# raulmur/ORB_SLAM2

Measured on NVIDIA H100. Metric: stereo frames/sec (ORB extract L+R + ComputeStereoMatches, KITTI-shaped 1242x375 @2000 kpts), higher is better.
Workload: dtype u8

## Files before the change

### orb_slam2_b200/csrc/borb_host.cu

```cuda
#include <cmath>
#include <cstdarg>
#include <cstdio>
#include <algorithm>
#include <cstdlib>
#include <cstring>

#include "borb_internal.h"

namespace borb {

static thread_local std::string tl_error;
void set_error(const char* fmt, ...) {
    char buf[512];
    va_list ap;
    va_start(ap, fmt);
    vsnprintf(buf, sizeof(buf), fmt, ap);
    va_end(ap);
    tl_error = buf;
}

std::atomic<int> g_poison{-1};

bool allow_max_smem(const void* func) {
    static std::mutex mu;
// ... 150 lines not shown
        v.inv_scale = e->inv_scale[l];
        v.patch_size = (float)(int)(PATCH * e->scale[l]);
        g.blur_base[l] = btile;
        btile += ((v.w + BLUR_TILE_W - 1) / BLUR_TILE_W) * ((v.h + BLUR_TILE_H - 1) / BLUR_TILE_H);
        if (l > 0) {
            const int wpad = (v.w + 8 + 3) & ~3;
            v.xtab_off = (unsigned)(tabs.size() / 4);
            resize_table(g.lv[l - 1].w, v.w, true, wpad - v.w, tabs);
            v.ytab_off = (unsigned)(tabs.size() / 4);
            resize_table(g.lv[l - 1].h, v.h, false, 0, tabs);
            v.xwin_off = (unsigned)(tabs.size() / 4);
            std::vector<int16_t> win;
            v.x_windowed = resize_window_table(tabs, (size_t)v.xtab_off * 4, wpad, win) ? 1 : 0;
            tabs.insert(tabs.end(), win.begin(), win.end());
        }
        if (quadtree_smem_bytes(v.node_cap) > 200 * 1024) {
            set_error("per-level quota %d exceeds the quadtree kernel's shared-memory envelope", v.quota);
            return BORB_ERR_UNSUPPORTED;
        }
    }
    g.blur_base[L] = btile;
    g.blur_tiles = btile;
    g.fast_blocks = blk;
    g.pyr_image_stride = (unsigned)align_up((int)pyr_off, g.lv[0].pitch);
    g.cand_image_stride = cand_off;
    g.sel_image_stride = sel_off;
    if (sel_off >= 65536) { set_error("keypoint capacity %d exceeds 65535", sel_off); return BORB_ERR_UNSUPPORTED; }
    return BORB_OK;
}

void free_workspace(Workspace& ws) {
    cudaFree(ws.pyr); cudaFree(ws.blur); cudaFree(ws.cand); cudaFree(ws.cand_cnt); cudaFree(ws.pnode); cudaFree(ws.sel);
    cudaFree(ws.sel_cnt); cudaFree(ws.kps); cudaFree(ws.desc); cudaFree(ws.nkp); cudaFree(ws.u_right); cudaFree(ws.depth);
    cudaFree(ws.sad); cudaFree(ws.tabs); cudaFree(ws.brief_slots); cudaFree(ws.pair_idx); cudaFree(ws.st_bins); cudaFree(ws.st_recs); cudaFree(ws.stage);
    free(ws.fast_tmaps); cudaFree(ws.fast_tiles);
    ws = Workspace();
}

borb_status ensure(borb_extractor* e, int w, int h, int n_images) {
    if (w < 1 || h < 1 || w > BORB_MAX_DIM || h > BORB_MAX_DIM) { set_error("image size %dx%d outside [1,%d]", w, h, BORB_MAX_DIM); return BORB_ERR_UNSUPPORTED; }
    BORB_CUDA(cudaSetDevice(e->device));
    const bool same_shape = e->have_geom && e->geom.w == w && e->geom.h == h;
    if (same_shape && e->ws.max_images >= n_images) return BORB_OK;
    BORB_CUDA(cudaStreamSynchronize(e->stream));
    std::vector<int16_t> tabs;
    e->have_geom = false;
    e->last_n_images = 0;
    e->last_stereo_pairs = 0;
    borb_status st = build_geometry(e, w, h, tabs);
    if (st != BORB_OK) return st;
    size_t n = (size_t)(n_images > 2 ? n_images : 2);
    if (same_shape && (size_t)e->ws.max_images > n) n = (size_t)e->ws.max_images;
    free_workspace(e->ws);
    if (e->h_counts) { cudaFreeHost(e->h_counts); e->h_counts = nullptr; }
    e->pair_cache.clear();
    const Geometry& g = e->geom;
    Workspace& ws = e->ws;
    BORB_CUDA(cudaMalloc(&ws.pyr, n * g.pyr_image_stride + 256));
    BORB_CUDA(cudaMalloc(&ws.blur, n * g.pyr_image_stride + 256));
    BORB_CUDA(cudaMalloc(&ws.cand, n * g.cand_image_stride * sizeof(uint32_t)));
    BORB_CUDA(cudaMalloc(&ws.pnode, n * g.cand_image_stride * sizeof(int)));
    BORB_CUDA(cudaMalloc(&ws.cand_cnt, n * g.nlevels * sizeof(int)));
    BORB_CUDA(cudaMalloc(&ws.sel, n * g.sel_image_stride * sizeof(uint32_t)));
    BORB_CUDA(cudaMalloc(&ws.sel_cnt, n * g.nlevels * sizeof(int)));
    BORB_CUDA(cudaMalloc(&ws.kps, n * g.sel_image_stride * sizeof(borb_keypoint)));
    BORB_CUDA(cudaMalloc(&ws.desc, n * g.sel_image_stride * 32));
    BORB_CUDA(cudaMalloc(&ws.nkp, n * sizeof(int)));
    BORB_CUDA(cudaMalloc(&ws.u_right, n * g.sel_image_stride * sizeof(float)));
    BORB_CUDA(cudaMalloc(&ws.depth, n * g.sel_image_stride * sizeof(float)));
    BORB_CUDA(cudaMalloc(&ws.sad, n * g.sel_image_stride * sizeof(int)));
    BORB_CUDA(cudaMalloc(&ws.pair_idx, n * 2 * sizeof(int)));
    BORB_CUDA(cudaMalloc(&ws.st_bins, n * stereo_bins_bytes_per_pair()));
    ws.st_recs_bytes = n * (size_t)stereo_rec_stride(g) * stereo_rec_bytes();
    BORB_CUDA(cudaMalloc(&ws.st_recs, ws.st_recs_bytes));
    BORB_CUDA(cudaMalloc(&ws.tabs, (tabs.size() + 4) * sizeof(int16_t)));
    BORB_CUDA(cudaMemcpy(ws.tabs, tabs.data(), tabs.size() * sizeof(int16_t), cudaMemcpyHostToDevice));
    const std::vector<uint32_t>& slots = brief_slot_table();
    BORB_CUDA(cudaMalloc(&ws.brief_slots, slots.size() * sizeof(uint32_t)));
    BORB_CUDA(cudaMemcpy(ws.brief_slots, slots.data(), slots.size() * sizeof(uint32_t), cudaMemcpyHostToDevice));
    BORB_CUDA(cudaMemset(ws.nkp, 0, n * sizeof(int)));
    BORB_CUDA(cudaMallocHost(&e->h_counts, n * 2 * sizeof(int)));
    ws.max_images = (int)n;
    ws.fast_tmaps = malloc(fast_tmaps_bytes());
    if ((st = build_fast_tmaps(g, ws, ws.fast_tmaps)) != BORB_OK) return st;
    if ((st = build_fast_tiles(g, ws)) != BORB_OK) return st;
    e->have_geom = true;
    return BORB_OK;
}

borb_status poison_extract(borb_extractor* e) {
    const int p = poison_byte();
    if (p < 0) return BORB_OK;
    const Geometry& g = e->geom;
    Workspace& ws = e->ws;
    const size_t n = (size_t)ws.max_images;
    cudaStream_t s = e->stream;
    if (ws.stage) BORB_CUDA(cudaMemsetAsync(ws.stage, p, ws.stage_bytes, s));
    BORB_CUDA(cudaMemsetAsync(ws.pyr, p, n * g.pyr_image_stride + 256, s));
    BORB_CUDA(cudaMemsetAsync(ws.blur, p, n * g.pyr_image_stride + 256, s));
    BORB_CUDA(cudaMemsetAsync(ws.cand, p, n * g.cand_image_stride * sizeof(uint32_t), s));
    BORB_CUDA(cudaMemsetAsync(ws.pnode, p, n * g.cand_image_stride * sizeof(int), s));
    BORB_CUDA(cudaMemsetAsync(ws.cand_cnt, p, n * g.nlevels * sizeof(int), s));
    BORB_CUDA(cudaMemsetAsync(ws.sel, p, n * g.sel_image_stride * sizeof(uint32_t), s));
    BORB_CUDA(cudaMemsetAsync(ws.sel_cnt, p, n * g.nlevels * sizeof(int), s));
    BORB_CUDA(cudaMemsetAsync(ws.kps, p, n * g.sel_image_stride * sizeof(borb_keypoint), s));
    BORB_CUDA(cudaMemsetAsync(ws.desc, p, n * g.sel_image_stride * 32, s));
    BORB_CUDA(cudaMemsetAsync(ws.nkp, p, n * sizeof(int), s));
    return BORB_OK;
}

borb_status poison_stereo(borb_extractor* e) {
    const int p = poison_byte();
    if (p < 0) return BORB_OK;
    Workspace& ws = e->ws;
    const size_t n = (size_t)ws.max_images * e->geom.sel_image_stride;
    cudaStream_t s = e->stream;
    BORB_CUDA(cudaMemsetAsync(ws.u_right, p, n * sizeof(float), s));
    BORB_CUDA(cudaMemsetAsync(ws.depth, p, n * sizeof(float), s));
    BORB_CUDA(cudaMemsetAsync(ws.sad, p, n * sizeof(int), s));
    BORB_CUDA(cudaMemsetAsync(ws.st_bins, p, (size_t)ws.max_images * stereo_bins_bytes_per_pair(), s));
    BORB_CUDA(cudaMemsetAsync(ws.st_recs, p, ws.st_recs_bytes, s));
    return BORB_OK;
}

void drain_timing(borb_extractor* e);
void begin_step(borb_extractor* e) {
    if (!e->timing) return;
    if (e->ev.empty()) {
        e->ev.resize((size_t)borb_extractor::EV_RING * 9);
        for (auto& x : e->ev) cudaEventCreate(&x);
    }
    if (e->ev_pending >= borb_extractor::EV_RING) {
        cudaStreamSynchronize(e->stream);
        drain_timing(e);
    }
    e->ev_slot = (e->ev_slot + 1) % borb_extractor::EV_RING;
    e->ev_mask[e->ev_slot] = 0;
    e->ev_pending++;
}
void mark(borb_extractor* e, int i) {
    if (!e->timing || e->ev.empty()) return;
    cudaEventRecord(e->ev[(size_t)e->ev_slot * 9 + i], e->stream);
    e->ev_mask[e->ev_slot] |= 1u << i;
}
void drain_timing(borb_extractor* e) {
    const int R = borb_extractor::EV_RING;
    for (int k = e->ev_pending - 1; k >= 0; k--) {
        const int slot = ((e->ev_slot - k) % R + R) % R;
        const unsigned m = e->ev_mask[slot];
        for (int i = 0; i < 8; i++) {
            float ms = 0.f;
            if (m & (1u << i)) {
                int j = i + 1;
                while (j < 9 && !(m & (1u << j))) j++;
// ... 147 lines not shown
    return BORB_OK;
}

borb_status enqueue_stereo(borb_extractor* eL, borb_extractor* eR, int n_pairs, const int* left_idx, const int* right_idx,
                           float bf, float b) {
    borb_extractor* e = eL;
    const Geometry& g = e->geom;
    std::vector<int> idx(2 * (size_t)n_pairs);
    for (int p = 0; p < n_pairs; p++) {
        idx[2 * p] = left_idx ? left_idx[p] : (eL == eR ? 2 * p : 0);
        idx[2 * p + 1] = right_idx ? right_idx[p] : (eL == eR ? 2 * p + 1 : 0);
        if (idx[2 * p] < 0 || idx[2 * p] >= eL->last_n_images || idx[2 * p + 1] < 0 || idx[2 * p + 1] >= eR->last_n_images) {
            set_error("stereo pair %d refers to an image outside the last batch", p);
            return BORB_ERR_STATE;
        }
    }
    if (n_pairs > e->ws.max_images) { set_error("too many pairs"); return BORB_ERR_INVALID_ARG; }
    if (idx != e->pair_cache) {
        BORB_CUDA(cudaStreamSynchronize(e->stream));
        std::memcpy(e->h_counts, idx.data(), idx.size() * sizeof(int));
        BORB_CUDA(cudaMemcpyAsync(e->ws.pair_idx, e->h_counts, idx.size() * sizeof(int), cudaMemcpyHostToDevice, e->stream));
        e->pair_cache = idx;
    }
    const int rec_stride = stereo_rec_stride(eR->geom);
    const size_t rec_bytes = (size_t)n_pairs * rec_stride * stereo_rec_bytes();
    if (rec_bytes > e->ws.st_recs_bytes) {
        BORB_CUDA(cudaStreamSynchronize(e->stream));
        cudaFree(e->ws.st_recs);
        e->ws.st_recs = nullptr;
        e->ws.st_recs_bytes = 0;
        BORB_CUDA(cudaMalloc(&e->ws.st_recs, rec_bytes));
        e->ws.st_recs_bytes = rec_bytes;
    }
    const borb_status pst = poison_stereo(e);
    if (pst != BORB_OK) return pst;
    StereoView L{eL->ws.pyr, eL->ws.kps, eL->ws.desc, eL->ws.nkp, eL->geom.pyr_image_stride, eL->geom.sel_image_stride};
    StereoView R{eR->ws.pyr, eR->ws.kps, eR->ws.desc, eR->ws.nkp, eR->geom.pyr_image_stride, eR->geom.sel_image_stride};
    mark(e, 6);
    e->launches += launch_stereo(g, L, R, e->ws.pair_idx, n_pairs, bf, b, e->ws.u_right, e->ws.depth, e->ws.sad, g.sel_image_stride,
                                 e->ws.st_bins, e->ws.st_recs, rec_stride, e->stream);
    mark(e, 7);
    BORB_CUDA(cudaGetLastError());
    e->last_stereo_pairs = (eL == eR && !left_idx && !right_idx) ? n_pairs : 0;
    return BORB_OK;
}

borb_status download_stereo(borb_extractor* e, int n_pairs, float* u_right, float* depth, int cap) {
    const Geometry& g = e->geom;
    const int m = cap < g.sel_image_stride ? cap : g.sel_image_stride;
    if (u_right && m > 0)
        BORB_CUDA(cudaMemcpy2DAsync(u_right, (size_t)cap * 4, e->ws.u_right, (size_t)g.sel_image_stride * 4, (size_t)m * 4, n_pairs, cudaMemcpyDeviceToHost, e->stream));
    if (depth && m > 0)
        BORB_CUDA(cudaMemcpy2DAsync(depth, (size_t)cap * 4, e->ws.depth, (size_t)g.sel_image_stride * 4, (size_t)m * 4, n_pairs, cudaMemcpyDeviceToHost, e->stream));
    return BORB_OK;
}

borb_status finish_timing(borb_extractor* e) {
    if (e->timing && e->ev_pending > 0) drain_timing(e);
    return BORB_OK;
}

}

const std::vector<uint32_t>& brief_slot_table() {
    static const std::vector<uint32_t> table = [] {
        std::vector<uint32_t> t((size_t)BRIEF_BINS * 512);
        int row[512], col[512], order[512];
        for (int b = 0; b < BRIEF_BINS; b++) {
            const double th = (b + 0.5) * (2.0 * 3.14159265358979323846 / BRIEF_BINS);
            const double a = std::cos(th), s = std::sin(th);
            for (int p = 0; p < 512; p++) {
                const int x = kPattern[2 * p], y = kPattern[2 * p + 1];
                row[p] = (int)std::lround(x * s + y * a);
// ... 513 lines not shown
```

### orb_slam2_b200/csrc/borb_internal.h

```cpp
#pragma once
#include <cuda_runtime.h>
#include <stdint.h>

#include <atomic>
#include <mutex>
#include <string>
#include <vector>

#include "../../include/borb.h"

namespace borb {

extern std::atomic<int> g_poison;
inline int poison_byte() { return g_poison.load(std::memory_order_relaxed); }

constexpr int EDGE = 19;
constexpr int PATCH = 31;
constexpr int HALF_PATCH = 15;
constexpr int MIN_BORDER = 16;
constexpr int TH_HIGH = 100;
constexpr int TH_LOW = 50;
constexpr int BLUR_TILE_W = 120;
constexpr int BLUR_TILE_H = 64;
constexpr int FAST_TILE_W = 124;
// ... 40 lines not shown
    int ini_th, min_th;
    int fast_mode;
    int fast_blocks;
    unsigned pyr_image_stride;
    unsigned cand_image_stride;
    int sel_image_stride;
    int blur_tiles;
    int blur_base[BORB_MAX_LEVELS + 1];
    int umax[16];
    LevelGeom lv[BORB_MAX_LEVELS];
};

struct Workspace {
    int max_images = 0;
    uint8_t* pyr = nullptr;
    uint8_t* blur = nullptr;
    uint32_t* cand = nullptr;
    int* cand_cnt = nullptr;
    int* pnode = nullptr;
    uint32_t* sel = nullptr;
    int* sel_cnt = nullptr;
    borb_keypoint* kps = nullptr;
    uint8_t* desc = nullptr;
    int* nkp = nullptr;
    float* u_right = nullptr;
    float* depth = nullptr;
    int* sad = nullptr;
    int16_t* tabs = nullptr;
    uint32_t* brief_slots = nullptr;
    int* pair_idx = nullptr;
    int* st_bins = nullptr;
    void* st_recs = nullptr;
    size_t st_recs_bytes = 0;
    uint8_t* stage = nullptr;
    size_t stage_bytes = 0;
    void* fast_tmaps = nullptr;
    void* fast_tiles = nullptr;
    int fast_n_tiles = 0;
};

constexpr int BRIEF_BINS = 32;
const std::vector<uint32_t>& brief_slot_table();

void set_error(const char* fmt, ...);
bool allow_max_smem(const void* func);
#define BORB_CUDA(call)                                                                             \
    do {                                                                                            \
        cudaError_t _e = (call);                                                                    \
        if (_e != cudaSuccess) {                                                                    \
            borb::set_error("%s failed: %s (%s:%d)", #call, cudaGetErrorString(_e), __FILE__, __LINE__); \
            return (_e == cudaErrorNoDevice || _e == cudaErrorInsufficientDriver) ? BORB_ERR_NO_DEVICE : BORB_ERR_CUDA; \
        }                                                                                           \
    } while (0)

int launch_repack_remap(const Geometry& g, const Workspace& ws, const uint8_t* stage, int src_stride, size_t src_image_bytes, int src_w,
                        int src_h, const float* mx0, const float* my0, const float* mx1, const float* my1, int n_images, cudaStream_t s);
int launch_repack_color(const Geometry& g, const Workspace& ws, const uint8_t* stage, int src_stride, size_t src_image_bytes, int channels,
                        int rgb, int n_images, cudaStream_t s);
int launch_repack(const Geometry& g, const Workspace& ws, const uint8_t* stage, int src_stride, size_t src_image_bytes,
                  int n_images, cudaStream_t s);
int launch_pyramid(const Geometry& g, const Workspace& ws, int n_images, cudaStream_t s);
int launch_fast(const Geometry& g, const Workspace& ws, int n_images, cudaStream_t s);
int launch_quadtree(const Geometry& g, const Workspace& ws, int n_images, cudaStream_t s);
int launch_blur(const Geometry& g, const Workspace& ws, int n_images, cudaStream_t s);
int launch_describe(const Geometry& g, const Workspace& ws, int n_images, cudaStream_t s);
int launch_describe_math_probe(int fn, const float* a, const float* b, int n, float* out, cudaStream_t s);
int launch_match_math_probe(int fn, const float* a, const float* b, int n, float log_scale, int n_levels, void* out,
                            cudaStream_t s);

struct StereoView {
    const uint8_t* pyr;
    const borb_keypoint* kps;
    const uint8_t* desc;
    const int* nkp;
    unsigned pyr_image_stride;
    int kp_image_stride;
};
int launch_stereo(const Geometry& g, const StereoView& L, const StereoView& R, const int* d_pair_idx, int n_pairs,
                  float bf, float b, float* d_u_right, float* d_depth, int* d_sad, int out_stride, int* d_bins, void* d_recs,
                  int rec_stride, cudaStream_t s);
int stereo_rec_stride(const Geometry& g);
size_t stereo_bins_bytes_per_pair();
size_t stereo_rec_bytes();
size_t quadtree_smem_bytes(int node_cap);
borb_status build_fast_tmaps(const Geometry& g, const Workspace& ws, void* out_tmaps);
borb_status build_fast_tiles(const Geometry& g, Workspace& ws);
size_t fast_tmaps_bytes();

}

struct borb_extractor {
    borb_extractor_cfg cfg;
    int device = 0;
    cudaStream_t stream = nullptr;
    std::vector<float> scale, inv_scale, sigma2, inv_sigma2;
    std::vector<int> per_level;
    int umax[16];
    bool have_geom = false;
    borb::Geometry geom;
    borb::Workspace ws;
    int last_n_images = 0;
    int last_stereo_pairs = 0;
    int in_channels = 1;
    int in_rgb = 1;
    float* d_map[2][2] = {{nullptr, nullptr}, {nullptr, nullptr}};
    int map_src_w = 0, map_src_h = 0, map_dst_w = 0, map_dst_h = 0;
    int fast_mode = 0;
    uint64_t launches = 0;
    static constexpr int EV_RING = 128;
    bool timing = false;
    std::vector<cudaEvent_t> ev;
    unsigned ev_mask[EV_RING] = {};
    int ev_slot = 0;
    int ev_pending = 0;
    float stage_ms[8] = {};
    double stage_sum_ms[8] = {};
// ... 5 lines not shown
```

### orb_slam2_b200/csrc/k_stereo.cu

```cuda
#include "borb_internal.h"

namespace borb {

namespace {

__device__ __forceinline__ int hamming256(const uint4 a0, const uint4 a1, const uint4* __restrict__ b) {
    const uint4 b0 = b[0], b1 = b[1];
    return __popc(a0.x ^ b0.x) + __popc(a0.y ^ b0.y) + __popc(a0.z ^ b0.z) + __popc(a0.w ^ b0.w) +
           __popc(a1.x ^ b1.x) + __popc(a1.y ^ b1.y) + __popc(a1.z ^ b1.z) + __popc(a1.w ^ b1.w);
}

}

constexpr int SBIN_SHIFT = 3;
constexpr int SBIN_MAX = 512;
struct __align__(16) RightRec { int iR; int band; int octave; float x; };

__global__ void __launch_bounds__(256) stereo_bin_kernel(const __grid_constant__ Geometry g, StereoView Rv,
                                                         const int* __restrict__ pair_idx, int* __restrict__ bin_start,
                                                         RightRec* __restrict__ recs, int rec_stride) {
    __shared__ int cnt[SBIN_MAX + 1];
    __shared__ int wsum[40];
    const int pair = blockIdx.x, tid = threadIdx.x;
    const int imR = pair_idx[2 * pair + 1];
    const int nR = Rv.nkp[imR];
    const int nb = min((g.h >> SBIN_SHIFT) + 1, SBIN_MAX);
    const borb_keypoint* kR = Rv.kps + (size_t)imR * Rv.kp_image_stride;
    for (int i = tid; i <= nb; i += 256) cnt[i] = 0;
    __syncthreads();
    for (int i = tid; i < nR; i += 256) {
        const borb_keypoint kr = kR[i];
        const float r = __fmul_rn(2.0f, g.lv[kr.octave].scale);
        const int maxr = (int)ceilf(__fadd_rn(kr.y, r)), minr = (int)floorf(__fsub_rn(kr.y, r));
        const int b0 = max(minr, 0) >> SBIN_SHIFT, b1 = min(min(maxr, g.h - 1) >> SBIN_SHIFT, nb - 1);
        for (int b = b0; b <= b1; b++) atomicAdd(&cnt[b], 1);
    }
    __syncthreads();
    {
        const int lane = tid & 31, w = tid >> 5;
        const int i0 = 2 * tid, i1 = 2 * tid + 1;
        const int c0 = i0 < nb ? cnt[i0] : 0, c1 = i1 < nb ? cnt[i1] : 0;
        int incl = c0 + c1;
#pragma unroll
        for (int off = 1; off < 32; off <<= 1) {
            const int t = __shfl_up_sync(0xFFFFFFFFu, incl, off);
            if (lane >= off) incl += t;
        }
        if (lane == 31) wsum[w] = incl;
        __syncthreads();
        if (w == 0) {
            int v = lane < 8 ? wsum[lane] : 0, inc2 = v;
#pragma unroll
            for (int off = 1; off < 8; off <<= 1) {
                const int t = __shfl_up_sync(0xFFFFFFFFu, inc2, off);
                if (lane >= off) inc2 += t;
            }
            if (lane < 8) wsum[8 + lane] = inc2 - v;
            if (lane == 7) wsum[16] = inc2;
        }
        __syncthreads();
        const int base = wsum[8 + w] + incl - (c0 + c1);
        if (i0 < nb) cnt[i0] = base;
        if (i1 < nb) cnt[i1] = base + c0;
        if (tid == 0) cnt[nb] = wsum[16];
        __syncthreads();
    }
    int* bs = bin_start + (size_t)pair * (SBIN_MAX + 1);
    for (int i = tid; i <= nb; i += 256) bs[i] = cnt[i];
    __syncthreads();
    RightRec* out = recs + (size_t)pair * rec_stride;
    for (int i = tid; i < nR; i += 256) {
        const borb_keypoint kr = kR[i];
        const float r = __fmul_rn(2.0f, g.lv[kr.octave].scale);
        const int maxr = (int)ceilf(__fadd_rn(kr.y, r)), minr = (int)floorf(__fsub_rn(kr.y, r));
        const int b0 = max(minr, 0) >> SBIN_SHIFT, b1 = min(min(maxr, g.h - 1) >> SBIN_SHIFT, nb - 1);
        RightRec rec;
        rec.iR = i; rec.band = (minr & 0xFFFF) | (maxr << 16); rec.octave = kr.octave; rec.x = kr.x;
        for (int b = b0; b <= b1; b++) {
            const int pos = atomicAdd(&cnt[b], 1);
            if (pos < rec_stride) out[pos] = rec;
        }
    }
}

__global__ void __launch_bounds__(256, 6) stereo_match_kernel(const __grid_constant__ Geometry g, StereoView Lv, StereoView Rv,
                                                           const int* __restrict__ pair_idx, float bf, float b,
                                                           float* __restrict__ u_right, float* __restrict__ depth,
                                                           int* __restrict__ sad, int out_stride,
                                                           const int* __restrict__ bin_start, const RightRec* __restrict__ recs,
                                                           int rec_stride) {
    const int pair = blockIdx.y;
    const int imL = pair_idx[2 * pair], imR = pair_idx[2 * pair + 1];
    const int lane = threadIdx.x & 31;
    const int iL = blockIdx.x * (blockDim.x >> 5) + (threadIdx.x >> 5);
    const int nL = Lv.nkp[imL], nR = Rv.nkp[imR];
    if (iL >= nL) return;
    const size_t o = (size_t)pair * out_stride + iL;
    const borb_keypoint* kL = Lv.kps + (size_t)imL * Lv.kp_image_stride;
    const borb_keypoint* kR = Rv.kps + (size_t)imR * Rv.kp_image_stride;
    const uint8_t* dL = Lv.desc + (size_t)imL * Lv.kp_image_stride * 32;
    const uint8_t* dR = Rv.desc + (size_t)imR * Rv.kp_image_stride * 32;

    float uR_out = -1.0f, depth_out = -1.0f;
    int sad_out = -1;

    const borb_keypoint kp = kL[iL];
    const int levelL = kp.octave;
    const float vL = kp.y, uL = kp.x;
    const float maxD = __fdiv_rn(bf, b);
    const float minU = __fsub_rn(uL, maxD), maxU = uL;
    const int row = (int)vL;
    const uint4 a0 = reinterpret_cast<const uint4*>(dL + (size_t)iL * 32)[0];
    const uint4 a1 = reinterpret_cast<const uint4*>(dL + (size_t)iL * 32)[1];
    unsigned best = ((unsigned)TH_HIGH << 16);
    if (!(maxU < 0) && row >= 0 && row < g.h) {
        const int nb = min((g.h >> SBIN_SHIFT) + 1, SBIN_MAX);
        const int bin = min(row >> SBIN_SHIFT, nb - 1);
        const int* bs = bin_start + (size_t)pair * (SBIN_MAX + 1);
        const int e0 = bs[bin], e1 = min(bs[bin + 1], rec_stride);
        const RightRec* rr = recs + (size_t)pair * rec_stride;
        for (int e = e0 + lane; e < e1; e += 32) {
            const RightRec rc = rr[e];
            const int minr = (int)(short)(rc.band & 0xFFFF), maxr = rc.band >> 16;
            if (row < minr || row > maxr) continue;
            if (rc.octave < levelL - 1 || rc.octave > levelL + 1) continue;
            if (rc.x >= minU && rc.x <= maxU) {
                const int dist = hamming256(a0, a1, reinterpret_cast<const uint4*>(dR + (size_t)rc.iR * 32));
                const unsigned key = ((unsigned)dist << 16) | (unsigned)rc.iR;
                best = min(best, key);
            }
        }
    }
#pragma unroll
    for (int off = 16; off > 0; off >>= 1) best = min(best, __shfl_xor_sync(0xFFFFFFFFu, best, off));
    const int bestDist = (int)(best >> 16);
    const int thOrbDist = (TH_HIGH + TH_LOW) / 2;
    if (bestDist < thOrbDist) {
        const int bestIdxR = (int)(best & 0xFFFFu);
        const float uR0 = kR[bestIdxR].x;
        const LevelGeom& LG = g.lv[levelL];
        const float sf = LG.inv_scale;
        const int scaleduL = (int)roundf(__fmul_rn(kp.x, sf));
        const int scaledvL = (int)roundf(__fmul_rn(kp.y, sf));
        const int scaleduR0 = (int)roundf(__fmul_rn(uR0, sf));
        const int w = 5, Lh = 5;
        const int iniu = scaleduR0 + Lh - w, endu = scaleduR0 + Lh + w + 1;
        const bool ok = !(iniu < 0 || endu >= LG.w) && scaleduR0 - Lh - w >= 0 && scaledvL - w >= 0 &&
                        scaledvL + w < LG.h && scaleduL - w >= 0 && scaleduL + w < LG.w;
        if (ok) {
            const uint8_t* IL = Lv.pyr + (size_t)imL * Lv.pyr_image_stride + LG.pyr_off;
            const uint8_t* IR = Rv.pyr + (size_t)imR * Rv.pyr_image_stride + LG.pyr_off;
            const int cL = IL[(size_t)scaledvL * LG.pitch + scaleduL];
            int il[4];
            int offs[4];
#pragma unroll
            for (int k = 0; k < 4; k++) {
                const int e = lane + 32 * k;
                if (e < 121) {
                    const int yy = e / 11, xx = e - yy * 11;
                    offs[k] = (scaledvL - w + yy) * LG.pitch + (xx - w);
                    il[k] = (int)IL[offs[k] + scaleduL] - cL;
                } else { offs[k] = -1; il[k] = 0; }
            }
            int bestD = 0x7FFFFFFF, bestinc = 0;
            int dists[11];
#pragma unroll
            for (int inc = -5; inc <= 5; inc++) {
                const int uc = scaleduR0 + inc;
                const int cR = IR[(size_t)scaledvL * LG.pitch + uc];
                int s = 0;
#pragma unroll
                for (int k = 0; k < 4; k++)
                    if (offs[k] >= 0) s += abs(il[k] - ((int)IR[offs[k] + uc] - cR));
#pragma unroll
                for (int off = 16; off > 0; off >>= 1) s += __shfl_xor_sync(0xFFFFFFFFu, s, off);
                dists[inc + 5] = s;
                if (s < bestD) { bestD = s; bestinc = inc; }
            }
            if (!(bestinc == -Lh || bestinc == Lh)) {
                float d1 = 0.f, d2 = 0.f, d3 = 0.f;
#pragma unroll
                for (int i = 1; i < 10; i++)
                    if (i == bestinc + 5) { d1 = (float)dists[i - 1]; d2 = (float)dists[i]; d3 = (float)dists[i + 1]; }
                const float num = __fsub_rn(d1, d3);
                const float den = __fmul_rn(2.0f, __fsub_rn(__fadd_rn(d1, d3), __fmul_rn(2.0f, d2)));
                const float deltaR = __fdiv_rn(num, den);
                if (!(deltaR < -1.f || deltaR > 1.f)) {
                    float bestuR = __fmul_rn(LG.scale, __fadd_rn(__fadd_rn((float)scaleduR0, (float)bestinc), deltaR));
                    float disparity = __fsub_rn(uL, bestuR);
                    if (disparity >= 0.f && disparity < maxD) {
                        if (disparity <= 0.f) {
                            disparity = 0.01f;
                            bestuR = (float)((double)uL - 0.01);
                        }
                        depth_out = __fdiv_rn(bf, disparity);
                        uR_out = bestuR;
                        sad_out = bestD;
                    }
                }
            }
        }
    }
    if (lane == 0) {
        u_right[o] = uR_out;
        depth[o] = depth_out;
        sad[o] = sad_out;
    }
}

__global__ void __launch_bounds__(256) stereo_median_kernel(StereoView Lv, const int* __restrict__ pair_idx,
                                                            float* __restrict__ u_right, float* __restrict__ depth,
                                                            const int* __restrict__ sad, int out_stride) {
    __shared__ int hist[256];
    __shared__ int sel[3];
    const int pair = blockIdx.x;
    const int nL = Lv.nkp[pair_idx[2 * pair]];
    const size_t o = (size_t)pair * out_stride;
    const int tid = threadIdx.x;
    hist[tid] = 0;
    __syncthreads();
    int cnt = 0;
    for (int i = tid; i < nL; i += 256) {
        const int d = sad[o + i];
        if (d >= 0) { atomicAdd(&hist[min(d >> 8, 255)], 1); cnt++; }
    }
    __shared__ int tot;
    if (tid == 0) tot = 0;
    __syncthreads();
    if (cnt) atomicAdd(&tot, cnt);
    __syncthreads();
    const int n = tot;
    if (n == 0) return;
    const int kth = n / 2;
    if (tid == 0) {
        int acc = 0, bin = 0;
        for (; bin < 256; bin++) { if (acc + hist[bin] > kth) break; acc += hist[bin]; }
        sel[0] = bin; sel[1] = kth - acc;
    }
    __syncthreads();
    const int hiBin = sel[0], rem = sel[1];
    __syncthreads();
    hist[tid] = 0;
    __syncthreads();
    for (int i = tid; i < nL; i += 256) {
        const int d = sad[o + i];
        if (d >= 0 && min(d >> 8, 255) == hiBin) atomicAdd(&hist[d & 255], 1);
    }
    __syncthreads();
    if (tid == 0) {
        int acc = 0, bin = 0;
        for (; bin < 256; bin++) { if (acc + hist[bin] > rem) break; acc += hist[bin]; }
        sel[2] = (hiBin << 8) | bin;
    }
    __syncthreads();
    const float median = (float)sel[2];
    const float thDist = __fmul_rn(1.5f * 1.4f, median);
    for (int i = tid; i < nL; i += 256) {
        const int d = sad[o + i];
        if (d >= 0 && !((float)d < thDist)) { u_right[o + i] = -1.0f; depth[o + i] = -1.0f; }
    }
}

int stereo_rec_stride(const Geometry& g) {
    const int band = 2 * (int)ceilf(2.0f * g.lv[g.nlevels - 1].scale) + 3;
    return g.sel_image_stride * ((band >> SBIN_SHIFT) + 2);
}
size_t stereo_bins_bytes_per_pair() { return (size_t)(SBIN_MAX + 1) * sizeof(int); }
size_t stereo_rec_bytes() { return sizeof(RightRec); }

int launch_stereo(const Geometry& g, const StereoView& L, const StereoView& R, const int* d_pair_idx, int n_pairs,
                  float bf, float b, float* d_u_right, float* d_depth, int* d_sad, int out_stride, int* d_bins, void* d_recs,
                  int rec_stride, cudaStream_t s) {
    stereo_bin_kernel<<<n_pairs, 256, 0, s>>>(g, R, d_pair_idx, d_bins, reinterpret_cast<RightRec*>(d_recs), rec_stride);
    dim3 grid((g.sel_image_stride + 7) / 8, n_pairs);
    stereo_match_kernel<<<grid, 256, 0, s>>>(g, L, R, d_pair_idx, bf, b, d_u_right, d_depth, d_sad, out_stride, d_bins,
                                             reinterpret_cast<const RightRec*>(d_recs), rec_stride);
    stereo_median_kernel<<<n_pairs, 256, 0, s>>>(L, d_pair_idx, d_u_right, d_depth, d_sad, out_stride);
    return 3;
}

}
```

Before: 44100.

## Parallelize stereo binning across chunks and vectorize SAD window search

Splits the single-block-per-pair right-keypoint binning into a chunked count kernel and a chunked fill kernel with per-chunk prefix offsets, so binning uses many blocks instead of one. Right records shrink to 8 bytes with packed metadata, and the match loop batches four record loads per lane and tracks the best x. The SAD patch search is rewritten with packed 16-bit byte-perm and viaddmax/viaddmin arithmetic plus a warp-shuffle reduction, and the median kernel replaces serial thread-0 scans with a block scan. It adds one kernel launch and an extra scratch buffer, and the packed SAD logic carries correctness risk.

```diff
diff --git a/orb_slam2_b200/csrc/borb_host.cu b/orb_slam2_b200/csrc/borb_host.cu
--- a/orb_slam2_b200/csrc/borb_host.cu
+++ b/orb_slam2_b200/csrc/borb_host.cu
@@ -206,7 +206,7 @@
 void free_workspace(Workspace& ws) {
     cudaFree(ws.pyr); cudaFree(ws.blur); cudaFree(ws.cand); cudaFree(ws.cand_cnt); cudaFree(ws.pnode); cudaFree(ws.sel);
     cudaFree(ws.sel_cnt); cudaFree(ws.kps); cudaFree(ws.desc); cudaFree(ws.nkp); cudaFree(ws.u_right); cudaFree(ws.depth);
-    cudaFree(ws.sad); cudaFree(ws.tabs); cudaFree(ws.brief_slots); cudaFree(ws.pair_idx); cudaFree(ws.st_bins); cudaFree(ws.st_recs); cudaFree(ws.stage);
+    cudaFree(ws.sad); cudaFree(ws.tabs); cudaFree(ws.brief_slots); cudaFree(ws.pair_idx); cudaFree(ws.st_bins); cudaFree(ws.st_recs); cudaFree(ws.st_chunk_cnt); cudaFree(ws.stage);
     free(ws.fast_tmaps); cudaFree(ws.fast_tiles);
     ws = Workspace();
 }
@@ -247,6 +247,8 @@
     BORB_CUDA(cudaMalloc(&ws.st_bins, n * stereo_bins_bytes_per_pair()));
     ws.st_recs_bytes = n * (size_t)stereo_rec_stride(g) * stereo_rec_bytes();
     BORB_CUDA(cudaMalloc(&ws.st_recs, ws.st_recs_bytes));
+    ws.st_chunk_cnt_bytes = n * stereo_chunk_cnt_bytes_per_pair(g);
+    BORB_CUDA(cudaMalloc(&ws.st_chunk_cnt, ws.st_chunk_cnt_bytes));
     BORB_CUDA(cudaMalloc(&ws.tabs, (tabs.size() + 4) * sizeof(int16_t)));
     BORB_CUDA(cudaMemcpy(ws.tabs, tabs.data(), tabs.size() * sizeof(int16_t), cudaMemcpyHostToDevice));
     const std::vector<uint32_t>& slots = brief_slot_table();
@@ -294,6 +296,7 @@
     BORB_CUDA(cudaMemsetAsync(ws.sad, p, n * sizeof(int), s));
     BORB_CUDA(cudaMemsetAsync(ws.st_bins, p, (size_t)ws.max_images * stereo_bins_bytes_per_pair(), s));
     BORB_CUDA(cudaMemsetAsync(ws.st_recs, p, ws.st_recs_bytes, s));
+    BORB_CUDA(cudaMemsetAsync(ws.st_chunk_cnt, p, ws.st_chunk_cnt_bytes, s));
     return BORB_OK;
 }
 
@@ -507,13 +510,22 @@
         BORB_CUDA(cudaMalloc(&e->ws.st_recs, rec_bytes));
         e->ws.st_recs_bytes = rec_bytes;
     }
+    const size_t cnt_bytes = (size_t)n_pairs * stereo_chunk_cnt_bytes_per_pair(eR->geom);
+    if (cnt_bytes > e->ws.st_chunk_cnt_bytes) {
+        BORB_CUDA(cudaStreamSynchronize(e->stream));
+        cudaFree(e->ws.st_chunk_cnt);
+        e->ws.st_chunk_cnt = nullptr;
+        e->ws.st_chunk_cnt_bytes = 0;
+        BORB_CUDA(cudaMalloc(&e->ws.st_chunk_cnt, cnt_bytes));
+        e->ws.st_chunk_cnt_bytes = cnt_bytes;
+    }
     const borb_status pst = poison_stereo(e);
     if (pst != BORB_OK) return pst;
     StereoView L{eL->ws.pyr, eL->ws.kps, eL->ws.desc, eL->ws.nkp, eL->geom.pyr_image_stride, eL->geom.sel_image_stride};
     StereoView R{eR->ws.pyr, eR->ws.kps, eR->ws.desc, eR->ws.nkp, eR->geom.pyr_image_stride, eR->geom.sel_image_stride};
     mark(e, 6);
     e->launches += launch_stereo(g, L, R, e->ws.pair_idx, n_pairs, bf, b, e->ws.u_right, e->ws.depth, e->ws.sad, g.sel_image_stride,
-                                 e->ws.st_bins, e->ws.st_recs, rec_stride, e->stream);
+                                 e->ws.st_bins, e->ws.st_recs, rec_stride, e->ws.st_chunk_cnt, e->stream);
     mark(e, 7);
     BORB_CUDA(cudaGetLastError());
     e->last_stereo_pairs = (eL == eR && !left_idx && !right_idx) ? n_pairs : 0;
diff --git a/orb_slam2_b200/csrc/borb_internal.h b/orb_slam2_b200/csrc/borb_internal.h
--- a/orb_slam2_b200/csrc/borb_internal.h
+++ b/orb_slam2_b200/csrc/borb_internal.h
@@ -96,6 +96,8 @@
     int* st_bins = nullptr;
     void* st_recs = nullptr;
     size_t st_recs_bytes = 0;
+    int* st_chunk_cnt = nullptr;
+    size_t st_chunk_cnt_bytes = 0;
     uint8_t* stage = nullptr;
     size_t stage_bytes = 0;
     void* fast_tmaps = nullptr;
@@ -142,10 +144,11 @@
 };
 int launch_stereo(const Geometry& g, const StereoView& L, const StereoView& R, const int* d_pair_idx, int n_pairs,
                   float bf, float b, float* d_u_right, float* d_depth, int* d_sad, int out_stride, int* d_bins, void* d_recs,
-                  int rec_stride, cudaStream_t s);
+                  int rec_stride, int* d_chunk_cnt, cudaStream_t s);
 int stereo_rec_stride(const Geometry& g);
 size_t stereo_bins_bytes_per_pair();
 size_t stereo_rec_bytes();
+size_t stereo_chunk_cnt_bytes_per_pair(const Geometry& g);
 size_t quadtree_smem_bytes(int node_cap);
 borb_status build_fast_tmaps(const Geometry& g, const Workspace& ws, void* out_tmaps);
 borb_status build_fast_tiles(const Geometry& g, Workspace& ws);
diff --git a/orb_slam2_b200/csrc/k_stereo.cu b/orb_slam2_b200/csrc/k_stereo.cu
--- a/orb_slam2_b200/csrc/k_stereo.cu
+++ b/orb_slam2_b200/csrc/k_stereo.cu
@@ -10,78 +10,127 @@
            __popc(a1.x ^ b1.x) + __popc(a1.y ^ b1.y) + __popc(a1.z ^ b1.z) + __popc(a1.w ^ b1.w);
 }
 
+__device__ __forceinline__ int block_excl_scan256(int v, int* wsum, int& total) {
+    const int lane = threadIdx.x & 31, w = threadIdx.x >> 5;
+    int incl = v;
+#pragma unroll
+    for (int off = 1; off < 32; off <<= 1) {
+        const int t = __shfl_up_sync(0xFFFFFFFFu, incl, off);
+        if (lane >= off) incl += t;
+    }
+    if (lane == 31) wsum[w] = incl;
+    __syncthreads();
+    if (w == 0) {
+        const int x = lane < 8 ? wsum[lane] : 0;
+        int inc2 = x;
+#pragma unroll
+        for (int off = 1; off < 8; off <<= 1) {
+            const int t = __shfl_up_sync(0xFFFFFFFFu, inc2, off);
+            if (lane >= off) inc2 += t;
+        }
+        if (lane < 8) wsum[8 + lane] = inc2 - x;
+        if (lane == 7) wsum[16] = inc2;
+    }
+    __syncthreads();
+    total = wsum[16];
+    return wsum[8 + w] + incl - v;
+}
+
 }
 
 constexpr int SBIN_SHIFT = 3;
 constexpr int SBIN_MAX = 512;
-struct __align__(16) RightRec { int iR; int band; int octave; float x; };
-
-__global__ void __launch_bounds__(256) stereo_bin_kernel(const __grid_constant__ Geometry g, StereoView Rv,
-                                                         const int* __restrict__ pair_idx, int* __restrict__ bin_start,
-                                                         RightRec* __restrict__ recs, int rec_stride) {
-    __shared__ int cnt[SBIN_MAX + 1];
-    __shared__ int wsum[40];
-    const int pair = blockIdx.x, tid = threadIdx.x;
+constexpr int SBIN_CHUNK = 256;
+struct __align__(8) RightRec { unsigned meta; float x; };
+static_assert(BORB_MAX_DIM <= (SBIN_MAX << SBIN_SHIFT), "a row's bin must not be clamped");
+
+__device__ __forceinline__ int stereo_nbins(const Geometry& g) { return min((g.h >> SBIN_SHIFT) + 1, SBIN_MAX); }
+
+__device__ __forceinline__ void right_band(const Geometry& g, float y, int octave, int nb, int& minr, int& maxr, int& b0, int& b1) {
+    const float r = __fmul_rn(2.0f, g.lv[octave].scale);
+    maxr = (int)ceilf(__fadd_rn(y, r));
+    minr = (int)floorf(__fsub_rn(y, r));
+    b0 = max(minr, 0) >> SBIN_SHIFT;
+    b1 = min(min(maxr, g.h - 1) >> SBIN_SHIFT, nb - 1);
+}
+
+__global__ void __launch_bounds__(SBIN_CHUNK) stereo_bin_count_kernel(const __grid_constant__ Geometry g, StereoView Rv,
+                                                                      const int* __restrict__ pair_idx, int* __restrict__ chunk_cnt,
+                                                                      int n_chunks) {
+    __shared__ int cnt[SBIN_MAX];
+    const int pair = blockIdx.y, chunk = blockIdx.x, tid = threadIdx.x;
     const int imR = pair_idx[2 * pair + 1];
     const int nR = Rv.nkp[imR];
-    const int nb = min((g.h >> SBIN_SHIFT) + 1, SBIN_MAX);
-    const borb_keypoint* kR = Rv.kps + (size_t)imR * Rv.kp_image_stride;
-    for (int i = tid; i <= nb; i += 256) cnt[i] = 0;
-    __syncthreads();
-    for (int i = tid; i < nR; i += 256) {
-        const borb_keypoint kr = kR[i];
-        const float r = __fmul_rn(2.0f, g.lv[kr.octave].scale);
-        const int maxr = (int)ceilf(__fadd_rn(kr.y, r)), minr = (int)floorf(__fsub_rn(kr.y, r));
-        const int b0 = max(minr, 0) >> SBIN_SHIFT, b1 = min(min(maxr, g.h - 1) >> SBIN_SHIFT, nb - 1);
+    if (chunk * SBIN_CHUNK >= nR) return;
+    const int nb = stereo_nbins(g);
+    for (int i = tid; i < nb; i += SBIN_CHUNK) cnt[i] = 0;
+    __syncthreads();
+    const int i = chunk * SBIN_CHUNK + tid;
+    if (i < nR) {
+        const borb_keypoint* kr = Rv.kps + (size_t)imR * Rv.kp_image_stride + i;
+        int minr, maxr, b0, b1;
+        right_band(g, kr->y, kr->octave, nb, minr, maxr, b0, b1);
         for (int b = b0; b <= b1; b++) atomicAdd(&cnt[b], 1);
     }
     __syncthreads();
-    {
-        const int lane = tid & 31, w = tid >> 5;
-        const int i0 = 2 * tid, i1 = 2 * tid + 1;
-        const int c0 = i0 < nb ? cnt[i0] : 0, c1 = i1 < nb ? cnt[i1] : 0;
-        int incl = c0 + c1;
-#pragma unroll
-        for (int off = 1; off < 32; off <<= 1) {
-            const int t = __shfl_up_sync(0xFFFFFFFFu, incl, off);
-            if (lane >= off) incl += t;
+    int* out = chunk_cnt + ((size_t)pair * n_chunks + chunk) * SBIN_MAX;
+    for (int b = tid; b < nb; b += SBIN_CHUNK) out[b] = cnt[b];
+}
+
+__global__ void __launch_bounds__(SBIN_CHUNK) stereo_bin_fill_kernel(const __grid_constant__ Geometry g, StereoView Rv,
+                                                                     const int* __restrict__ pair_idx, const int* __restrict__ chunk_cnt,
+                                                                     int n_chunks, int* __restrict__ bin_start,
+                                                                     RightRec* __restrict__ recs, int rec_stride) {
+    __shared__ int base[SBIN_MAX];
+    __shared__ int wsum[17];
+    const int pair = blockIdx.y, chunk = blockIdx.x, tid = threadIdx.x;
+    const int imR = pair_idx[2 * pair + 1];
+    const int nR = Rv.nkp[imR];
+    const int used = (nR + SBIN_CHUNK - 1) / SBIN_CHUNK;
+    if (chunk > 0 && chunk >= used) return;
+    const int nb = stereo_nbins(g);
+    const int i0 = 2 * tid;
+    int tot0 = 0, tot1 = 0, pre0 = 0, pre1 = 0;
+    if (i0 < nb) {
+        const int* cc = chunk_cnt + (size_t)pair * n_chunks * SBIN_MAX + i0;
+        for (int c = 0; c < used; c++) {
+            const int2 v = *reinterpret_cast<const int2*>(cc + (size_t)c * SBIN_MAX);
+            const int v1 = i0 + 1 < nb ? v.y : 0;
+            tot0 += v.x; tot1 += v1;
+            if (c < chunk) { pre0 += v.x; pre1 += v1; }
         }
-        if (lane == 31) wsum[w] = incl;
-        __syncthreads();
-        if (w == 0) {
-            int v = lane < 8 ? wsum[lane] : 0, inc2 = v;
-#pragma unroll
-            for (int off = 1; off < 8; off <<= 1) {
-                const int t = __shfl_up_sync(0xFFFFFFFFu, inc2, off);
-                if (lane >= off) inc2 += t;
-            }
-            if (lane < 8) wsum[8 + lane] = inc2 - v;
-            if (lane == 7) wsum[16] = inc2;
-        }
-        __syncthreads();
-        const int base = wsum[8 + w] + incl - (c0 + c1);
-        if (i0 < nb) cnt[i0] = base;
-        if (i1 < nb) cnt[i1] = base + c0;
-        if (tid == 0) cnt[nb] = wsum[16];
-        __syncthreads();
-    }
-    int* bs = bin_start + (size_t)pair * (SBIN_MAX + 1);
-    for (int i = tid; i <= nb; i += 256) bs[i] = cnt[i];
-    __syncthreads();
+    }
+    int total;
+    const int excl = block_excl_scan256(tot0 + tot1, wsum, total);
+    if (i0 < nb) base[i0] = excl + pre0;
+    if (i0 + 1 < nb) base[i0 + 1] = excl + tot0 + pre1;
+    if (chunk == 0) {
+        int* bs = bin_start + (size_t)pair * (SBIN_MAX + 1);
+        if (i0 < nb) bs[i0] = excl;
+        if (i0 + 1 < nb) bs[i0 + 1] = excl + tot0;
+        if (tid == 0) bs[nb] = total;
+    }
+    __syncthreads();
+    const int i = chunk * SBIN_CHUNK + tid;
+    if (i >= nR) return;
+    const borb_keypoint* kr = Rv.kps + (size_t)imR * Rv.kp_image_stride + i;
+    const int octave = kr->octave;
+    RightRec rec;
+    rec.x = kr->x;
+    int minr, maxr, b0, b1;
+    right_band(g, kr->y, octave, nb, minr, maxr, b0, b1);
     RightRec* out = recs + (size_t)pair * rec_stride;
-    for (int i = tid; i < nR; i += 256) {
-        const borb_keypoint kr = kR[i];
-        const float r = __fmul_rn(2.0f, g.lv[kr.octave].scale);
-        const int maxr = (int)ceilf(__fadd_rn(kr.y, r)), minr = (int)floorf(__fsub_rn(kr.y, r));
-        const int b0 = max(minr, 0) >> SBIN_SHIFT, b1 = min(min(maxr, g.h - 1) >> SBIN_SHIFT, nb - 1);
-        RightRec rec;
-        rec.iR = i; rec.band = (minr & 0xFFFF) | (maxr << 16); rec.octave = kr.octave; rec.x = kr.x;
-        for (int b = b0; b <= b1; b++) {
-            const int pos = atomicAdd(&cnt[b], 1);
-            if (pos < rec_stride) out[pos] = rec;
-        }
-    }
-}
+    for (int b = b0; b <= b1; b++) {
+        const int lo = min(max(minr - (b << SBIN_SHIFT), -1), 8), hi = min(max(maxr - (b << SBIN_SHIFT), -1), 8);
+        rec.meta = (unsigned)i | (unsigned)octave << 16 | (unsigned)(lo + 1) << 20 | (unsigned)(hi + 1) << 24;
+        const int pos = atomicAdd(&base[b], 1);
+        if (pos < rec_stride) out[pos] = rec;
+    }
+}
+
+__device__ __forceinline__ uint32_t dup_byte(uint32_t w, int q) { return __byte_perm(w, 0u, 0x4040u | (unsigned)q | ((unsigned)q << 8)); }
+__device__ __forceinline__ uint32_t pair_lo(uint32_t w) { return __byte_perm(w, 0u, 0x4140u); }
+__device__ __forceinline__ uint32_t pair_hi(uint32_t w) { return __byte_perm(w, 0u, 0x4342u); }
 
 __global__ void __launch_bounds__(256, 6) stereo_match_kernel(const __grid_constant__ Geometry g, StereoView Lv, StereoView Rv,
                                                            const int* __restrict__ pair_idx, float bf, float b,
@@ -93,95 +142,146 @@
     const int imL = pair_idx[2 * pair], imR = pair_idx[2 * pair + 1];
     const int lane = threadIdx.x & 31;
     const int iL = blockIdx.x * (blockDim.x >> 5) + (threadIdx.x >> 5);
-    const int nL = Lv.nkp[imL], nR = Rv.nkp[imR];
+    const int nL = Lv.nkp[imL];
     if (iL >= nL) return;
     const size_t o = (size_t)pair * out_stride + iL;
-    const borb_keypoint* kL = Lv.kps + (size_t)imL * Lv.kp_image_stride;
-    const borb_keypoint* kR = Rv.kps + (size_t)imR * Rv.kp_image_stride;
+    const borb_keypoint* kpL = Lv.kps + (size_t)imL * Lv.kp_image_stride + iL;
     const uint8_t* dL = Lv.desc + (size_t)imL * Lv.kp_image_stride * 32;
     const uint8_t* dR = Rv.desc + (size_t)imR * Rv.kp_image_stride * 32;
+    const uint4 a0 = reinterpret_cast<const uint4*>(dL + (size_t)iL * 32)[0];
+    const uint4 a1 = reinterpret_cast<const uint4*>(dL + (size_t)iL * 32)[1];
 
     float uR_out = -1.0f, depth_out = -1.0f;
     int sad_out = -1;
 
-    const borb_keypoint kp = kL[iL];
-    const int levelL = kp.octave;
-    const float vL = kp.y, uL = kp.x;
+    const int levelL = kpL->octave;
+    const float vL = kpL->y, uL = kpL->x;
     const float maxD = __fdiv_rn(bf, b);
     const float minU = __fsub_rn(uL, maxD), maxU = uL;
     const int row = (int)vL;
-    const uint4 a0 = reinterpret_cast<const uint4*>(dL + (size_t)iL * 32)[0];
-    const uint4 a1 = reinterpret_cast<const uint4*>(dL + (size_t)iL * 32)[1];
+
     unsigned best = ((unsigned)TH_HIGH << 16);
+    float bestX = 0.f;
     if (!(maxU < 0) && row >= 0 && row < g.h) {
         const int nb = min((g.h >> SBIN_SHIFT) + 1, SBIN_MAX);
         const int bin = min(row >> SBIN_SHIFT, nb - 1);
         const int* bs = bin_start + (size_t)pair * (SBIN_MAX + 1);
         const int e0 = bs[bin], e1 = min(bs[bin + 1], rec_stride);
         const RightRec* rr = recs + (size_t)pair * rec_stride;
-        for (int e = e0 + lane; e < e1; e += 32) {
-            const RightRec rc = rr[e];
-            const int minr = (int)(short)(rc.band & 0xFFFF), maxr = rc.band >> 16;
-            if (row < minr || row > maxr) continue;
-            if (rc.octave < levelL - 1 || rc.octave > levelL + 1) continue;
-            if (rc.x >= minU && rc.x <= maxU) {
-                const int dist = hamming256(a0, a1, reinterpret_cast<const uint4*>(dR + (size_t)rc.iR * 32));
-                const unsigned key = ((unsigned)dist << 16) | (unsigned)rc.iR;
-                best = min(best, key);
+        const int rrow = (row - (bin << SBIN_SHIFT)) + 1;
+        for (int e = e0 + lane; e < e1; e += 128) {
+            RightRec rc[4];
+#pragma unroll
+            for (int t = 0; t < 4; t++)
+                if (e + 32 * t < e1) rc[t] = rr[e + 32 * t];
+#pragma unroll
+            for (int t = 0; t < 4; t++) {
+                if (e + 32 * t >= e1) continue;
+                const unsigned m = rc[t].meta;
+                const int octave = (int)(m >> 16) & 15, lo = (int)(m >> 20) & 15, hi = (int)(m >> 24) & 15;
+                if (rrow < lo || rrow > hi) continue;
+                if (octave < levelL - 1 || octave > levelL + 1) continue;
+                if (rc[t].x >= minU && rc[t].x <= maxU) {
+                    const unsigned iR = m & 0xFFFFu;
+                    const int dist = hamming256(a0, a1, reinterpret_cast<const uint4*>(dR + (size_t)iR * 32));
+                    const unsigned key = ((unsigned)dist << 16) | iR;
+                    if (key < best) { best = key; bestX = rc[t].x; }
+                }
             }
         }
     }
+    const unsigned mine = best;
 #pragma unroll
     for (int off = 16; off > 0; off >>= 1) best = min(best, __shfl_xor_sync(0xFFFFFFFFu, best, off));
     const int bestDist = (int)(best >> 16);
     const int thOrbDist = (TH_HIGH + TH_LOW) / 2;
+    const unsigned holder = __ballot_sync(0xFFFFFFFFu, mine == best);
+    const float uR0 = __shfl_sync(0xFFFFFFFFu, bestX, __ffs(holder) - 1);
     if (bestDist < thOrbDist) {
-        const int bestIdxR = (int)(best & 0xFFFFu);
-        const float uR0 = kR[bestIdxR].x;
         const LevelGeom& LG = g.lv[levelL];
         const float sf = LG.inv_scale;
-        const int scaleduL = (int)roundf(__fmul_rn(kp.x, sf));
-        const int scaledvL = (int)roundf(__fmul_rn(kp.y, sf));
+        const int scaleduL = (int)roundf(__fmul_rn(uL, sf));
+        const int scaledvL = (int)roundf(__fmul_rn(vL, sf));
         const int scaleduR0 = (int)roundf(__fmul_rn(uR0, sf));
         const int w = 5, Lh = 5;
         const int iniu = scaleduR0 + Lh - w, endu = scaleduR0 + Lh + w + 1;
         const bool ok = !(iniu < 0 || endu >= LG.w) && scaleduR0 - Lh - w >= 0 && scaledvL - w >= 0 &&
                         scaledvL + w < LG.h && scaleduL - w >= 0 && scaleduL + w < LG.w;
         if (ok) {
+            const int srow = min(lane >> 1, 10), half = lane & 1;
+            const size_t prow = (size_t)(scaledvL - w + srow) * LG.pitch;
             const uint8_t* IL = Lv.pyr + (size_t)imL * Lv.pyr_image_stride + LG.pyr_off;
+            const uint8_t* pl = IL + prow + (scaleduL - w + 6 * half);
+            const int lsh = 8 * (int)((uintptr_t)pl & 3);
+            const uint32_t* ql = reinterpret_cast<const uint32_t*>((uintptr_t)pl & ~(uintptr_t)3);
+            const uint32_t lw0 = ql[0], lw1 = ql[1], lw2 = ql[2];
+            const int cL = IL[(size_t)scaledvL * LG.pitch + scaleduL];
             const uint8_t* IR = Rv.pyr + (size_t)imR * Rv.pyr_image_stride + LG.pyr_off;
-            const int cL = IL[(size_t)scaledvL * LG.pitch + scaleduL];
-            int il[4];
-            int offs[4];
-#pragma unroll
-            for (int k = 0; k < 4; k++) {
-                const int e = lane + 32 * k;
-                if (e < 121) {
-                    const int yy = e / 11, xx = e - yy * 11;
-                    offs[k] = (scaledvL - w + yy) * LG.pitch + (xx - w);
-                    il[k] = (int)IL[offs[k] + scaleduL] - cL;
-                } else { offs[k] = -1; il[k] = 0; }
-            }
-            int bestD = 0x7FFFFFFF, bestinc = 0;
-            int dists[11];
-#pragma unroll
-            for (int inc = -5; inc <= 5; inc++) {
-                const int uc = scaleduR0 + inc;
-                const int cR = IR[(size_t)scaledvL * LG.pitch + uc];
-                int s = 0;
-#pragma unroll
-                for (int k = 0; k < 4; k++)
-                    if (offs[k] >= 0) s += abs(il[k] - ((int)IR[offs[k] + uc] - cR));
-#pragma unroll
-                for (int off = 16; off > 0; off >>= 1) s += __shfl_xor_sync(0xFFFFFFFFu, s, off);
-                dists[inc + 5] = s;
-                if (s < bestD) { bestD = s; bestinc = inc; }
-            }
+            const uint8_t* p = IR + prow + (scaleduR0 - Lh - w + 6 * half);
+            const int rsh = 8 * (int)((uintptr_t)p & 3);
+            const uint32_t* q = reinterpret_cast<const uint32_t*>((uintptr_t)p & ~(uintptr_t)3);
+            const uint32_t w0 = q[0], w1 = q[1], w2 = q[2], w3 = q[3], w4 = q[4];
+            const uint32_t ra0 = __funnelshift_r(w0, w1, rsh), ra1 = __funnelshift_r(w1, w2, rsh);
+            const uint32_t ra2 = __funnelshift_r(w2, w3, rsh), ra3 = __funnelshift_r(w3, w4, rsh);
+            const uint32_t ra4 = w4 >> rsh;
+            const uint32_t ra[4] = {ra0, ra1, ra2, ra3};
+            const uint32_t ro[4] = {__funnelshift_r(ra0, ra1, 8), __funnelshift_r(ra1, ra2, 8), __funnelshift_r(ra2, ra3, 8),
+                                    __funnelshift_r(ra3, ra4, 8)};
+            auto P = [&](int c) -> uint32_t {
+                const uint32_t x = (c & 1) ? ro[c >> 2] : ra[c >> 2];
+                return (c & 2) ? pair_hi(x) : pair_lo(x);
+            };
+            const uint32_t la0 = __funnelshift_r(lw0, lw1, lsh), la1 = __funnelshift_r(lw1, lw2, lsh);
+            const uint32_t biasL = (uint32_t)(255 - cL) * 0x10001u;
+            const uint32_t A[6] = {dup_byte(la0, 0) + biasL, dup_byte(la0, 1) + biasL, dup_byte(la0, 2) + biasL,
+                                   dup_byte(la0, 3) + biasL, dup_byte(la1, 0) + biasL, dup_byte(la1, 1) + biasL};
+            const uint32_t m5 = half == 0 ? 0xFFFFFFFFu : 0u;
+            uint32_t acc[6];
+#pragma unroll
+            for (int k = 0; k < 6; k++) {
+                const uint32_t biasR = 0x00FF00FFu - __shfl_sync(0xFFFFFFFFu, P(5 + 2 * k), 10);
+                uint32_t a = 0u;
+#pragma unroll
+                for (int j = 0; j < 6; j++) {
+                    const uint32_t mx = __viaddmax_u16x2(P(j + 2 * k), biasR, A[j]);
+                    const uint32_t mn = __viaddmin_u16x2(P(j + 2 * k), biasR, A[j]);
+                    a += j < 5 ? mx - mn : (mx - mn) & m5;
+                }
+                acc[k] = a;
+            }
+            const uint32_t lm = lane < 22 ? 0xFFFFFFFFu : 0u;
+            uint32_t v[4];
+#pragma unroll
+            for (int i = 0; i < 4; i++) {
+                const uint32_t lo = acc[i] & lm, hi = i < 2 ? acc[4 + i] & lm : 0u;
+                const bool up = lane & 16;
+                v[i] = (up ? hi : lo) + __shfl_xor_sync(0xFFFFFFFFu, up ? lo : hi, 16);
+            }
+            uint32_t u[2];
+#pragma unroll
+            for (int i = 0; i < 2; i++) {
+                const bool up = lane & 8;
+                u[i] = (up ? v[2 + i] : v[i]) + __shfl_xor_sync(0xFFFFFFFFu, up ? v[i] : v[2 + i], 8);
+            }
+            const bool up4 = lane & 4;
+            uint32_t W = (up4 ? u[1] : u[0]) + __shfl_xor_sync(0xFFFFFFFFu, up4 ? u[0] : u[1], 4);
+            W += __shfl_xor_sync(0xFFFFFFFFu, W, 2);
+            W += __shfl_xor_sync(0xFFFFFFFFu, W, 1);
+            const int k = lane >> 2;
+            unsigned key = k <= 5 ? ((W & 0xFFFFu) << 4) | (unsigned)(2 * k) : 0xFFFFFFFFu;
+            if (k < 5) key = min(key, ((W >> 16) << 4) | (unsigned)(2 * k + 1));
+            key = min(key, __shfl_xor_sync(0xFFFFFFFFu, key, 4));
+            key = min(key, __shfl_xor_sync(0xFFFFFFFFu, key, 8));
+            key = min(key, __shfl_xor_sync(0xFFFFFFFFu, key, 16));
+            const int bestD = (int)(key >> 4), sBest = (int)(key & 15u);
+            const int bestinc = sBest - Lh;
+            const int s1 = max(sBest - 1, 0), s3 = min(sBest + 1, 10);
+            const uint32_t W1 = __shfl_sync(0xFFFFFFFFu, W, (s1 >> 1) << 2);
+            const uint32_t W3 = __shfl_sync(0xFFFFFFFFu, W, (s3 >> 1) << 2);
             if (!(bestinc == -Lh || bestinc == Lh)) {
-                float d1 = 0.f, d2 = 0.f, d3 = 0.f;
-#pragma unroll
-                for (int i = 1; i < 10; i++)
-                    if (i == bestinc + 5) { d1 = (float)dists[i - 1]; d2 = (float)dists[i]; d3 = (float)dists[i + 1]; }
+                const float d1 = (float)(int)((s1 & 1) ? W1 >> 16 : W1 & 0xFFFFu);
+                const float d2 = (float)bestD;
+                const float d3 = (float)(int)((s3 & 1) ? W3 >> 16 : W3 & 0xFFFFu);
                 const float num = __fsub_rn(d1, d3);
                 const float den = __fmul_rn(2.0f, __fsub_rn(__fadd_rn(d1, d3), __fmul_rn(2.0f, d2)));
                 const float deltaR = __fdiv_rn(num, den);
@@ -212,48 +312,40 @@
                                                             float* __restrict__ u_right, float* __restrict__ depth,
                                                             const int* __restrict__ sad, int out_stride) {
     __shared__ int hist[256];
-    __shared__ int sel[3];
+    __shared__ int wsum[17];
+    __shared__ int sel[2];
     const int pair = blockIdx.x;
     const int nL = Lv.nkp[pair_idx[2 * pair]];
     const size_t o = (size_t)pair * out_stride;
     const int tid = threadIdx.x;
     hist[tid] = 0;
     __syncthreads();
-    int cnt = 0;
     for (int i = tid; i < nL; i += 256) {
         const int d = sad[o + i];
-        if (d >= 0) { atomicAdd(&hist[min(d >> 8, 255)], 1); cnt++; }
-    }
-    __shared__ int tot;
-    if (tid == 0) tot = 0;
-    __syncthreads();
-    if (cnt) atomicAdd(&tot, cnt);
-    __syncthreads();
-    const int n = tot;
+        if (d >= 0) atomicAdd(&hist[min(d >> 8, 255)], 1);
+    }
+    __syncthreads();
+    const int h = hist[tid];
+    int n;
+    const int acc = block_excl_scan256(h, wsum, n);
     if (n == 0) return;
     const int kth = n / 2;
-    if (tid == 0) {
-        int acc = 0, bin = 0;
-        for (; bin < 256; bin++) { if (acc + hist[bin] > kth) break; acc += hist[bin]; }
-        sel[0] = bin; sel[1] = kth - acc;
-    }
+    if (acc <= kth && kth < acc + h) { sel[0] = tid; sel[1] = kth - acc; }
+    hist[tid] = 0;
     __syncthreads();
     const int hiBin = sel[0], rem = sel[1];
-    __syncthreads();
-    hist[tid] = 0;
-    __syncthreads();
     for (int i = tid; i < nL; i += 256) {
         const int d = sad[o + i];
         if (d >= 0 && min(d >> 8, 255) == hiBin) atomicAdd(&hist[d & 255], 1);
     }
     __syncthreads();
-    if (tid == 0) {
-        int acc = 0, bin = 0;
-        for (; bin < 256; bin++) { if (acc + hist[bin] > rem) break; acc += hist[bin]; }
-        sel[2] = (hiBin << 8) | bin;
-    }
-    __syncthreads();
-    const float median = (float)sel[2];
+    const int h2 = hist[tid];
+    int n2;
+    const int acc2 = block_excl_scan256(h2, wsum, n2);
+    __shared__ int median_bits;
+    if (acc2 <= rem && rem < acc2 + h2) median_bits = (hiBin << 8) | tid;
+    __syncthreads();
+    const float median = (float)median_bits;
     const float thDist = __fmul_rn(1.5f * 1.4f, median);
     for (int i = tid; i < nL; i += 256) {
         const int d = sad[o + i];
@@ -267,16 +359,22 @@
 }
 size_t stereo_bins_bytes_per_pair() { return (size_t)(SBIN_MAX + 1) * sizeof(int); }
 size_t stereo_rec_bytes() { return sizeof(RightRec); }
+static int stereo_chunks(int kp_image_stride) { return (kp_image_stride + SBIN_CHUNK - 1) / SBIN_CHUNK; }
+size_t stereo_chunk_cnt_bytes_per_pair(const Geometry& g) { return (size_t)stereo_chunks(g.sel_image_stride) * SBIN_MAX * sizeof(int); }
 
 int launch_stereo(const Geometry& g, const StereoView& L, const StereoView& R, const int* d_pair_idx, int n_pairs,
                   float bf, float b, float* d_u_right, float* d_depth, int* d_sad, int out_stride, int* d_bins, void* d_recs,
-                  int rec_stride, cudaStream_t s) {
-    stereo_bin_kernel<<<n_pairs, 256, 0, s>>>(g, R, d_pair_idx, d_bins, reinterpret_cast<RightRec*>(d_recs), rec_stride);
+                  int rec_stride, int* d_chunk_cnt, cudaStream_t s) {
+    const int n_chunks = stereo_chunks(R.kp_image_stride);
+    const dim3 bin_grid(n_chunks, n_pairs);
+    stereo_bin_count_kernel<<<bin_grid, SBIN_CHUNK, 0, s>>>(g, R, d_pair_idx, d_chunk_cnt, n_chunks);
+    stereo_bin_fill_kernel<<<bin_grid, SBIN_CHUNK, 0, s>>>(g, R, d_pair_idx, d_chunk_cnt, n_chunks, d_bins,
+                                                           reinterpret_cast<RightRec*>(d_recs), rec_stride);
     dim3 grid((g.sel_image_stride + 7) / 8, n_pairs);
     stereo_match_kernel<<<grid, 256, 0, s>>>(g, L, R, d_pair_idx, bf, b, d_u_right, d_depth, d_sad, out_stride, d_bins,
                                              reinterpret_cast<const RightRec*>(d_recs), rec_stride);
     stereo_median_kernel<<<n_pairs, 256, 0, s>>>(L, d_pair_idx, d_u_right, d_depth, d_sad, out_stride);
-    return 3;
-}
-
-}
+    return 4;
+}
+
+}
```

Result: faster. 45160 (median of 6 runs) (+2.4%).
